# FrancisTheCat/raytracing_c

Measured on AMD Instinct MI355X. Metric: Mray/s, higher is better.
Workload: dtype f32; 1 GPU; helmet.glb 1920x1080, 256 spp, 8 bounces (BASELINE.json configs[2]); partition=single GPU

## Files before the change

include/rt_hip_diag.h:

```cpp
#ifndef RT_HIP_DIAG_H
#define RT_HIP_DIAG_H

#include "rt_hip.h"

#ifdef __cplusplus
extern "C" {
#endif

extern void rt_diag_set_tokens(void *disney_proc, void *debug_proc, void *background_proc);

extern void rt_diag_multi_fault(i32 no_peer, i32 failing_slot);

extern int  rt_set_pipeline(i32 pipeline);
extern i32  rt_get_pipeline(void);
extern void rt_set_wavefront_capacity(i64 records);

extern int rt_get_ledger(u64 *out, i32 n);
extern int rt_get_wave_times(u64 *out, i32 max_waves);
extern i64 rt_diag_device_bytes_live(void);
extern int rt_diag_release_staging(void);


extern int rt_test_math(i32 op, i32 n, f32 const *x, f32 const *y, f32 *out);
extern int rt_test_rcp_sweep(u64 out[6]);
extern int rt_test_srgb_sweep(u64 out[3]);
extern int rt_test_quantize_sweep(u64 out[2]);
extern int rt_test_group_sum(i32 group, i32 n_waves, u64 const *in, u8 const *valid, u64 *out);
extern int rt_test_sky_add_group(void);

extern int rt_test_trace(RT_Device_Scene *dscene, i32 n, f32 const *rays,
                         f32 *out_t, i32 *out_tri, f32 *out_uv);

extern int rt_test_trace_stream(RT_Device_Scene *dscene, i32 n, f32 const *rays, f32 const *pyramid, i32 exit_lanes, i32 mode,
                                f32 *out_t, i32 *out_tri, f32 *out_uv, u64 visits[2]);

extern int rt_test_tile_order(i32 n_tiles, u32 const *cost, u32 *order);

extern int rt_test_texture(RT_Device_Scene *dscene, i32 tex, i32 n, f32 const *uv, f32 *out_rgb);


extern int rt_test_shade(RT_Device_Scene *dscene, i32 mode, i32 n, i32 const *tri, f32 const *in, u32 const *state_in,
                         f32 *out, u32 *state_out, i32 *terminate, i32 *textured);
extern int rt_test_brdf(i32 n, f32 const *params, f32 const *in_dir, u32 const *state_in, f32 *out_dir, f32 *brdf, u32 *state_out);
extern int rt_test_background(RT_Device_Scene *dscene, i32 mode, i32 n, f32 const *dir, f32 *rgb);
extern int rt_test_primary_ray(Camera const *camera, i32 width, i32 height, i32 n, i32 const *xys, f32 *rays);

#ifdef __cplusplus
}
#endif

#endif
```

raytracing_c_amd/csrc/rt_dev.hip.h:

```cpp
#ifndef RT_DEV_HIP_H
#define RT_DEV_HIP_H

#include <hip/hip_runtime.h>
#include <stdint.h>

#include "rt_device.h"
#include "../../include/rt_math.h"

#define RT_BLOCK_WAVES 4
#define RT_BLOCK_THREADS (RT_BLOCK_WAVES * 64)

struct Ray3 {
  rt_v3 o, d;
  float inv_x, inv_y, inv_z;
  bool  fast;
};

__device__ __forceinline__ rt_v3 slab_bias3(const Ray3 &r) {
#ifdef RT_MATH_NO_FMA
  return rt_v3_make(0.0f, 0.0f, 0.0f);
#else
  float px, py, pz;
  asm volatile("v_mul_f32 %0, %1, %2" : "=v"(px) : "v"(r.o.x), "v"(r.inv_x));
  asm volatile("v_mul_f32 %0, %1, %2" : "=v"(py) : "v"(r.o.y), "v"(r.inv_y));
// ... 17 lines not shown
  LG_REGEN_X, LG_REGEN_L, LG_START_X, LG_START_L, LG_PRIM_X, LG_PRIM_L, LG_TILE_X, LG_JOIN_X, LG_FLUSH_X, LG_GRAB_X, LG_ROUND_X, LG_TRAV_CALLS,
  LG_NFULL_X, LG_NFULL_L, LG_NFULL_CAM, LG_NGLOB_X, LG_NGLOB_L, LG_NEXACT_X, LG_NEXACT_L, LG_CULLMASK_X, LG_PYRCHK_X, LG_NODE_WAIT_L,
  LG_NFEW0_X, LG_NFEW1_X, LG_NFEW2_X, LG_NFEW3_X, LG_NFEW4_X, LG_NFEW0_L, LG_NFEW1_L, LG_NFEW2_L, LG_NFEW3_L, LG_NFEW4_L,
  LG_LEAF_X, LG_LEAF_L, LG_LEAF_CAM, LG_POP_X, LG_POP_L, LG_POP_UP_L, LG_POP_RETEST_L, LG_POP_CAM, LG_POP_UP_X, LG_POP_RETEST_X, LG_POP_DONE_L,
  LG_CYC_S, LG_CYC_NODE, LG_CYC_LEAF, LG_CYC_POP, LG_CYC_WAVE, LG_CYC_TILE,
  LG_SKY_X, LG_SKY_L, LG_CYC_SKY,
  LG_CYC_COPY, LG_CYC_JOIN, LG_CYC_DRAIN, LG_DRAIN_X, LG_DRAIN_L, LG_CYC_FLUSH,
  LG_ROOT_FULL_X, LG_ROOT_FULL_L, LG_ROOT_CULL_X, LG_ROOT_CULL_L, LG_ROOT_LEFT_X, LG_ROOT_LEFT_L, LG_ROOTF_X, LG_ROOTF_L,
  LG_N
};
#define RT_LEDGER_ROW 128
#ifdef RT_LEDGER
__device__ __forceinline__ int lane_now();
__device__ __forceinline__ void lg_add(uint32_t *lg, int slot, uint32_t n) {
  if (lg && lane_now() == 0 && n != 0u) __hip_atomic_fetch_add(lg + slot, n, __ATOMIC_RELAXED, __HIP_MEMORY_SCOPE_AGENT);
}
#define LG(slot, n) lg_add(lg, (slot), (uint32_t)(n))
#define LG_ARG , lg
#else
#define LG(slot, n) ((void)0)
#define LG_ARG
#endif
#ifdef RT_LEDGER_MARKS
#define LGM(name) asm volatile("; LEDGER_MARK " name)
#else
#define LGM(name) ((void)0)
#endif
#if defined(RT_LEDGER) && RT_LEDGER >= 2
#define LGT0() const unsigned long long lg_t0 = __builtin_amdgcn_s_memtime()
#define LGT1(slot) LG((slot), (uint32_t)((__builtin_amdgcn_s_memtime() - lg_t0) >> 4))
#define LGD0(n_live) do { if (!lg_drain_t0) { lg_drain_t0 = __builtin_amdgcn_s_memtime(); LG(LG_DRAIN_X, 1); LG(LG_DRAIN_L, (n_live)); } } while (0)
#define LGD1() do { if (lg_drain_t0) { LG(LG_CYC_DRAIN, (uint32_t)((__builtin_amdgcn_s_memtime() - lg_drain_t0) >> 4)); lg_drain_t0 = 0ull; } } while (0)
#else
#define LGT0() ((void)0)
#define LGT1(slot) ((void)0)
#define LGD0(n_live) ((void)0)
#define LGD1() ((void)0)
#endif

__device__ __forceinline__ float4 ld4(const float *base, int idx4) {
  return reinterpret_cast<const float4 *>(base)[idx4];
}

typedef const float __attribute__((address_space(4))) cfloat;
__device__ __forceinline__ cfloat *as_scalar_ptr(const float *p) { return (cfloat *)(unsigned long long)p; }

__device__ __forceinline__ float as_f(int i) { return __int_as_float(i); }
__device__ __forceinline__ int   as_i(float f) { return __float_as_int(f); }


__device__ __forceinline__ float fmin_hw(float a, float b) { return __builtin_fminf(a, b); }
__device__ __forceinline__ float fmax_hw(float a, float b) { return __builtin_fmaxf(a, b); }

template <bool FAST>
__device__ __forceinline__ float slab_entry(const Ray3 &r, const rt_v3 &bs, float mnx, float mny, float mnz,
                                            float mxx, float mxy, float mxz, float t_max) {
  if (FAST) {
    float t0x = rt_slab_t_fast(mnx, r.o.x, r.inv_x, bs.x), t1x = rt_slab_t_fast(mxx, r.o.x, r.inv_x, bs.x);
    float t0y = rt_slab_t_fast(mny, r.o.y, r.inv_y, bs.y), t1y = rt_slab_t_fast(mxy, r.o.y, r.inv_y, bs.y);
    float t0z = rt_slab_t_fast(mnz, r.o.z, r.inv_z, bs.z), t1z = rt_slab_t_fast(mxz, r.o.z, r.inv_z, bs.z);
    float sx = fmin_hw(t0x, t1x), sy = fmin_hw(t0y, t1y), sz = fmin_hw(t0z, t1z);
    float bx = fmax_hw(t0x, t1x), by = fmax_hw(t0y, t1y), bz = fmax_hw(t0z, t1z);
    float t_minv = fmax_hw(RT_EPS, fmax_hw(sx, fmax_hw(sy, sz)));
    float t_maxv = fmin_hw(t_max, fmin_hw(bx, fmin_hw(by, bz)));
    return (t_minv < t_maxv) ? t_minv : RT_INF;
  } else {
    float t0x = rt_slab_t_exact(mnx, r.o.x, r.inv_x), t1x = rt_slab_t_exact(mxx, r.o.x, r.inv_x);
    float t0y = rt_slab_t_exact(mny, r.o.y, r.inv_y), t1y = rt_slab_t_exact(mxy, r.o.y, r.inv_y);
    float t0z = rt_slab_t_exact(mnz, r.o.z, r.inv_z), t1z = rt_slab_t_exact(mxz, r.o.z, r.inv_z);
    float sx = rt_min_ps(t0x, t1x), sy = rt_min_ps(t0y, t1y), sz = rt_min_ps(t0z, t1z);
    float bx = rt_max_ps(t0x, t1x), by = rt_max_ps(t0y, t1y), bz = rt_max_ps(t0z, t1z);
    float t_minv = rt_max_ps(RT_EPS, rt_max_ps(sx, rt_max_ps(sy, sz)));
    float t_maxv = rt_min_ps(t_max, rt_min_ps(bx, rt_min_ps(by, bz)));
    float e = (t_minv >= t_maxv) ? RT_INF : t_minv;
    return (e < t_max) ? e : RT_INF;
  }
}

template <bool FAST>
__device__ __forceinline__ float slab_entry_child(const float *n, const Ray3 &r) {
  float mnx = n[0], mny = n[8], mnz = n[16], mxx = n[24], mxy = n[32], mxz = n[40];
  if (FAST) {
    const rt_v3 bs = slab_bias3(r);
    float t0x = rt_slab_t_fast(mnx, r.o.x, r.inv_x, bs.x), t1x = rt_slab_t_fast(mxx, r.o.x, r.inv_x, bs.x);
    float t0y = rt_slab_t_fast(mny, r.o.y, r.inv_y, bs.y), t1y = rt_slab_t_fast(mxy, r.o.y, r.inv_y, bs.y);
    float t0z = rt_slab_t_fast(mnz, r.o.z, r.inv_z, bs.z), t1z = rt_slab_t_fast(mxz, r.o.z, r.inv_z, bs.z);
    float sx = fmin_hw(t0x, t1x), sy = fmin_hw(t0y, t1y), sz = fmin_hw(t0z, t1z);
    return fmax_hw(RT_EPS, fmax_hw(sx, fmax_hw(sy, sz)));
  }
  float t0x = rt_slab_t_exact(mnx, r.o.x, r.inv_x), t1x = rt_slab_t_exact(mxx, r.o.x, r.inv_x);
  float t0y = rt_slab_t_exact(mny, r.o.y, r.inv_y), t1y = rt_slab_t_exact(mxy, r.o.y, r.inv_y);
  float t0z = rt_slab_t_exact(mnz, r.o.z, r.inv_z), t1z = rt_slab_t_exact(mxz, r.o.z, r.inv_z);
  float sx = rt_min_ps(t0x, t1x), sy = rt_min_ps(t0y, t1y), sz = rt_min_ps(t0z, t1z);
  return rt_max_ps(RT_EPS, rt_max_ps(sx, rt_max_ps(sy, sz)));
}
__device__ __forceinline__ float slab_entry_child_any(const float *n, const Ray3 &r) {
  if (r.fast) return slab_entry_child<true>(n, r);
  return slab_entry_child<false>(n, r);
}

#define NODE_GLOBAL 0
#define NODE_SCALAR 1
#define NODE_LDS_ORDERED 3
#define RT_LDS_NODE_F4 13

static_assert(RT_LDS_NODE_F4 * 16 == RT_LDS_NODE_BYTES, "the host splits the LDS by the kernels' node stride (rt_device.h, lds_split)");

__device__ __forceinline__ int lds_node_f4(int node) { return (int)__umul24((unsigned)node, (unsigned)RT_LDS_NODE_F4); }

static inline int raise_lds_limit(const void *kernel, uint32_t *devices, int smem_bytes, int limit) {
  int dev = 0;
  (void)hipGetDevice(&dev);
  if (smem_bytes > 48 * 1024 && (dev >= 32 || !(__atomic_load_n(devices, __ATOMIC_RELAXED) & (1u << dev)))) {
    hipError_t e = hipFuncSetAttribute(kernel, hipFuncAttributeMaxDynamicSharedMemorySize, limit);
    if (e != hipSuccess) return (int)e;
    if (dev < 32) __atomic_fetch_or(devices, 1u << dev, __ATOMIC_RELAXED);
  }
  return 0;
}

template <bool FAST, int MODE>
__device__ __forceinline__ uint32_t node_enter(const RT_KParams &P, const Ray3 &r, int node, float hit_t,
                                               const float4 *lds_nodes) {
  int d[8];
  const rt_v3 bs = FAST ? slab_bias3(r) : rt_v3_make(0.0f, 0.0f, 0.0f);
  if (MODE == NODE_SCALAR) {
    cfloat *nb = as_scalar_ptr(P.nodes) + (size_t)node * 48;
#pragma unroll
    for (int k = 0; k < 8; k++) {
      d[k] = as_i(slab_entry<FAST>(r, bs, nb[k], nb[8 + k], nb[16 + k], nb[24 + k], nb[32 + k], nb[40 + k], hit_t));
    }
  } else if (MODE == NODE_LDS_ORDERED) {
    static_assert(FAST || MODE != NODE_LDS_ORDERED, "the ordered LDS form is for FAST rays only");
    const char *nbase = reinterpret_cast<const char *>(lds_nodes + lds_node_f4(node));
    const int nx = (as_i(r.inv_x) >> 31) & 96, ny = (as_i(r.inv_y) >> 31) & 96, nz = (as_i(r.inv_z) >> 31) & 96;
#pragma unroll
    for (int h = 0; h < 2; h++) {
      const float4 ax = *reinterpret_cast<const float4 *>(nbase + nx + h * 16), bx = *reinterpret_cast<const float4 *>(nbase + (96 - nx) + h * 16);
      const float4 ay = *reinterpret_cast<const float4 *>(nbase + 32 + ny + h * 16), by = *reinterpret_cast<const float4 *>(nbase + 32 + (96 - ny) + h * 16);
      const float4 az = *reinterpret_cast<const float4 *>(nbase + 64 + nz + h * 16), bz = *reinterpret_cast<const float4 *>(nbase + 64 + (96 - nz) + h * 16);
      const float nxs[4] = {ax.x, ax.y, ax.z, ax.w}, fxs[4] = {bx.x, bx.y, bx.z, bx.w};
      const float nys[4] = {ay.x, ay.y, ay.z, ay.w}, fys[4] = {by.x, by.y, by.z, by.w};
      const float nzs[4] = {az.x, az.y, az.z, az.w}, fzs[4] = {bz.x, bz.y, bz.z, bz.w};
#pragma unroll
      for (int k = 0; k < 4; k++) {
        const float sx = rt_slab_t_fast(nxs[k], r.o.x, r.inv_x, bs.x), bxx = rt_slab_t_fast(fxs[k], r.o.x, r.inv_x, bs.x);
        const float sy = rt_slab_t_fast(nys[k], r.o.y, r.inv_y, bs.y), byy = rt_slab_t_fast(fys[k], r.o.y, r.inv_y, bs.y);
        const float sz = rt_slab_t_fast(nzs[k], r.o.z, r.inv_z, bs.z), bzz = rt_slab_t_fast(fzs[k], r.o.z, r.inv_z, bs.z);
        const float t_minv = fmax_hw(RT_EPS, fmax_hw(sx, fmax_hw(sy, sz)));
        const float t_maxv = fmin_hw(hit_t, fmin_hw(bxx, fmin_hw(byy, bzz)));
        d[h * 4 + k] = as_i((t_minv < t_maxv) ? t_minv : RT_INF);
      }
    }
  } else {
    const float4 *nb = reinterpret_cast<const float4 *>(P.nodes) + (size_t)node * 12;
#pragma unroll
    for (int h = 0; h < 2; h++) {
      float4 mnx = nb[0 + h], mny = nb[2 + h], mnz = nb[4 + h];
      float4 mxx = nb[6 + h], mxy = nb[8 + h], mxz = nb[10 + h];
      d[h * 4 + 0] = as_i(slab_entry<FAST>(r, bs, mnx.x, mny.x, mnz.x, mxx.x, mxy.x, mxz.x, hit_t));
      d[h * 4 + 1] = as_i(slab_entry<FAST>(r, bs, mnx.y, mny.y, mnz.y, mxx.y, mxy.y, mxz.y, hit_t));
      d[h * 4 + 2] = as_i(slab_entry<FAST>(r, bs, mnx.z, mny.z, mnz.z, mxx.z, mxy.z, mxz.z, hit_t));
      d[h * 4 + 3] = as_i(slab_entry<FAST>(r, bs, mnx.w, mny.w, mnz.w, mxx.w, mxy.w, mxz.w, hit_t));
    }
  }

  int rank[8];
#pragma unroll
  for (int k = 0; k < 8; k++) rank[k] = k;
#pragma unroll
  for (int j = 0; j < 8; j++) {
#pragma unroll
    for (int k = j + 1; k < 8; k++) {
      int kb = (int)((uint32_t)(d[k] - d[j]) >> 31);
      rank[j] += kb;
      rank[k] -= kb;
    }
  }
  uint32_t w = 0, n_inf = 0;
#pragma unroll
  for (int j = 0; j < 8; j++) {
    int sh;
    asm("v_lshl_add_u32 %0, %1, 1, %1" : "=v"(sh) : "v"(rank[j]));
    w |= (uint32_t)j << sh;
    n_inf += ((uint32_t)d[j] + 0x00800000u) >> 31;
  }
  return w | ((8u - n_inf) << 24);
}

#define RT_SHORT_DIV_MAX_X 0x1p102f
__device__ __forceinline__ float rcp_exact(float x) {
  float xs = x * 0x1p24f;
  float y = __builtin_amdgcn_rcpf(xs);
  float e = __builtin_fmaf(-xs, y, 1.0f);
  float z = __builtin_fmaf(e, y, y);
  return __builtin_amdgcn_div_fixupf(z, xs, 1.0f) * 0x1p24f;
}
__device__ __forceinline__ float rcp_leaf(float x) {
  float xs = x * 0x1p24f;
  float y = __builtin_amdgcn_rcpf(xs);
  float e = __builtin_fmaf(-xs, y, 1.0f);
  float z = __builtin_fmaf(e, y, y);
  return z * 0x1p24f;
}
__device__ __forceinline__ bool rcp_exact_outside(float x) {
  return __builtin_fabsf(x) >= RT_SHORT_DIV_MAX_X && __builtin_fabsf(x) < RT_INF;
}

__device__ __forceinline__ rt_v3 normalize_dev(rt_v3 v) { return rt_v3_scale(v, rcp_exact(rt_sqrtf(rt_v3_dot(v, v)))); }

__device__ __forceinline__ unsigned long long accum_quantize_dev(float c) {
  float v = (c > 0.0f) ? c : 0.0f;
  v = (v > RT_ACCUM_MAX) ? RT_ACCUM_MAX : v;
  const uint32_t b = __float_as_uint(v);
  const uint32_t e = b >> 23;
  const unsigned long long m = (unsigned long long)((b & 0x007FFFFFu) | 0x00800000u) << 29;
  const uint32_t k = 147u - e;
  return m >> (k < 63u ? k : 63u);
}

__device__ __forceinline__ float tri_test(const Ray3 &r, float ax, float ay, float az, float e1x, float e1y, float e1z,
                                          float e2x, float e2y, float e2z, float &u_out, float &v_out) {
  rt_v3 a = rt_v3_make(ax, ay, az);
  rt_v3 edge1 = rt_v3_make(e1x, e1y, e1z);
  rt_v3 edge2 = rt_v3_make(e2x, e2y, e2z);
  rt_v3 rxe2 = rt_v3_cross(r.d, edge2);
  float det = rt_v3_dot(edge1, rxe2);
  float inv_det = 1.0f / det;
  rt_v3 s = rt_v3_sub(r.o, a);
  rt_v3 sxe1 = rt_v3_cross(s, edge1);
  float u = inv_det * rt_v3_dot(s, rxe2);
  float v = inv_det * rt_v3_dot(r.d, sxe1);
  float t = inv_det * rt_v3_dot(edge2, sxe1);
  bool miss = (u < -RT_EPS) || (u > 1.0f + RT_EPS) || (v < -RT_EPS) || (u + v > 1.0f + RT_EPS) || (t < RT_EPS);
  float dist = miss ? RT_INF : t;
  u_out = u;
  v_out = v;
  return (dist > 0.0f) ? dist : RT_INF;
}

// ... 1179 lines not shown
```

raytracing_c_amd/csrc/rt_diag.cpp:

```cpp

#include "rt_host.h"

#include <cmath>

#ifndef RT_DIAG_VARIANTS
#error rt_diag.cpp belongs to the diagnostic library only (-DRT_DIAG_VARIANTS)
#endif

extern "C" {
int rt_launch_test_math(int op, int n, const float *x, const float *y, float *out, hipStream_t stream);
int rt_launch_test_rcp_sweep(unsigned long long *counts, hipStream_t stream);
int rt_launch_test_srgb_sweep(unsigned long long *counts, hipStream_t stream);
int rt_launch_test_quantize_sweep(unsigned long long *counts, hipStream_t stream);
int rt_launch_test_sky_add_group(void);
int rt_launch_test_group_sum(int group, int n_waves, const unsigned long long *in, const unsigned char *valid, unsigned long long *out,
                              hipStream_t stream);
int rt_launch_test_trace(const RT_KParams *P, int n, const float *rays, float *out_t, int *out_tri, float *out_uv,
                         hipStream_t stream);
int rt_launch_test_trace_stream(const RT_KParams *P, int n, const float *rays, const float *pyr, int exit_lanes, int n_blocks,
                                int smem_bytes, float *out_t, int *out_tri, float *out_uv, unsigned long long *visits,
                                hipStream_t stream);
int rt_launch_test_texture(const RT_KParams *P, int tex, int n, const float *uv, float *out, hipStream_t stream);
int rt_launch_test_shade(const RT_KParams *P, int lds, int n, const int *tri, const float *in, const uint32_t *state_in, float *out,
                         uint32_t *state_out, int *terminate, int *textured, hipStream_t stream);
int rt_launch_test_brdf(int n, const float *params, const float *in_dir, const uint32_t *state_in, float *out_dir, float *brdf,
                        uint32_t *state_out, hipStream_t stream);
int rt_launch_test_background(const RT_KParams *P, int lds, int n, const float *dir, float *rgb, hipStream_t stream);
int rt_launch_test_primary_ray(const RT_KParams *P, int n, const int *xys, float *rays, hipStream_t stream);
int rt_wf_launch_camera(const RT_KParams *P, int n_blocks, int geometry, int smem_bytes, hipStream_t stream);
int rt_wf_launch_trace(const RT_KParams *P, int n_blocks, int geometry, int smem_bytes, hipStream_t stream);
int rt_wf_launch_shade(const RT_KParams *P, int n_blocks, int first, hipStream_t stream);
}

std::atomic<int>            g_pipeline{0};
static std::atomic<int64_t> g_wf_cap_records{(int64_t)96 << 20};

extern "C" int rt_set_pipeline(i32 pipeline) {
  if (pipeline != 0 && pipeline != 1) return rt_fail("rt_set_pipeline: %d is not 0 (tile stream) or 1 (wavefront)", pipeline);
  g_pipeline.store(pipeline);
  return 0;
}
extern "C" i32 rt_get_pipeline(void) { return g_pipeline.load(); }
extern "C" void rt_set_wavefront_capacity(i64 records) {
  if (records >= 1024) g_wf_cap_records.store(records);
}

extern "C" void rt_diag_set_tokens(void *disney, void *debug, void *background) {
  if (disney) g_tok_disney = (Shader_Proc)disney;
  if (debug) g_tok_debug = (Shader_Proc)debug;
  if (background) g_tok_background = (Background_Proc)background;
}

static int wavefront_ensure_queues(RT_Device_Scene *d, int64_t paths, int cam_waves, int max_waves) {
  const int64_t cap = g_wf_cap_records.load();
  const int64_t want = paths < cap ? paths : cap;
  const int64_t fill = WF_CHUNK - 63;
  const int64_t soft = (want + fill - 1) / fill + cam_waves + 1;
  if (d->wf_ctl && d->wf_soft0 >= soft && d->wf_waves >= max_waves) return 0;
  d->wf_hit0.reset(); d->wf_hit.reset(); d->wf_ray[0].reset(); d->wf_ray[1].reset(); d->wf_cnt.reset(); d->wf_ctl.reset();
  d->wf_soft0 = 0;
  const int64_t hard = soft + 2 * (int64_t)cam_waves + 8;
  const int64_t ray_chunks = (hard * WF_CHUNK + fill - 1) / fill + max_waves + 8;
  const int64_t hit_chunks = (ray_chunks * WF_CHUNK + fill - 1) / fill + max_waves + 8;
  HIP_TRY(d->wf_hit0.grow((size_t)hard * WF_HIT0_FIELDS * WF_CHUNK));
  HIP_TRY(d->wf_hit.grow((size_t)hit_chunks * WF_HIT_FIELDS * WF_CHUNK));
  HIP_TRY(d->wf_ray[0].grow((size_t)ray_chunks * WF_RAY_FIELDS * WF_CHUNK));
  HIP_TRY(d->wf_ray[1].grow((size_t)ray_chunks * WF_RAY_FIELDS * WF_CHUNK));
  HIP_TRY(d->wf_cnt.grow((size_t)(hard + hit_chunks + 2 * ray_chunks)));
  HIP_TRY(d->wf_ctl.grow((size_t)WF_N_CTL * WF_CTL_STRIDE));
// ... 116 lines not shown
  HIP_TRY(dout.grow((size_t)n));
  HIP_TRY(hipMemcpy(dx, x, bytes, hipMemcpyHostToDevice));
  if (y) {
    HIP_TRY(dy.grow((size_t)n));
    HIP_TRY(hipMemcpy(dy, y, bytes, hipMemcpyHostToDevice));
  }
  int rc = rt_launch_test_math(op, n, dx, dy, dout, nullptr);
  if (rc == 0) rc = (int)hipMemcpy(out, dout, bytes, hipMemcpyDeviceToHost);
  if (rc != 0) return rt_fail("rt_test_math failed: %s", hipGetErrorString((hipError_t)rc));
  return 0;
}

static int run_sweep(int (*launch)(unsigned long long *, hipStream_t), const char *name, u64 *out, int n_out) {
  Device &D = dev0();
  std::lock_guard<std::mutex> lock(D.mutex);
  if (ensure_device(D) != 0) return -1;
  if (!out) return rt_fail("%s: NULL", name);
  DevMem<unsigned long long> b;
  HIP_TRY(b.grow((size_t)n_out));
  HIP_TRY(hipMemset(b, 0, (size_t)n_out * sizeof(unsigned long long)));
  int rc = launch(b, nullptr);
  if (rc == 0) rc = (int)hipMemcpy(out, b, (size_t)n_out * sizeof(unsigned long long), hipMemcpyDeviceToHost);
  if (rc != 0) return rt_fail("%s failed: %s", name, hipGetErrorString((hipError_t)rc));
  return 0;
}

extern "C" int rt_test_rcp_sweep(u64 out[6]) { return run_sweep(rt_launch_test_rcp_sweep, "rt_test_rcp_sweep", out, 6); }

extern "C" int rt_test_srgb_sweep(u64 out[3]) { return run_sweep(rt_launch_test_srgb_sweep, "rt_test_srgb_sweep", out, 3); }

extern "C" int rt_test_quantize_sweep(u64 out[2]) { return run_sweep(rt_launch_test_quantize_sweep, "rt_test_quantize_sweep", out, 2); }

extern "C" int rt_test_group_sum(i32 group, i32 n_waves, u64 const *in, u8 const *valid, u64 *out) {
  Device &D = dev0();
  std::lock_guard<std::mutex> lock(D.mutex);
  if (ensure_device(D) != 0) return -1;
  if ((group != 4 && group != 16 && group != 64) || n_waves <= 0 || n_waves > 65535 || !in || !valid || !out)
    return rt_fail("rt_test_group_sum: bad arguments");
  const size_t n = (size_t)n_waves * 64;
  DevMem<unsigned long long> din, dout;
  DevMem<unsigned char> dvalid;
  HIP_TRY(din.grow(3 * n));
  HIP_TRY(dout.grow(3 * n));
  HIP_TRY(dvalid.grow(n));
  HIP_TRY(hipMemcpy(din, in, 3 * n * sizeof(u64), hipMemcpyHostToDevice));
  HIP_TRY(hipMemcpy(dvalid, valid, n, hipMemcpyHostToDevice));
  int rc = rt_launch_test_group_sum(group, n_waves, din, dvalid, dout, nullptr);
  if (rc == 0) rc = (int)hipMemcpy(out, dout, 3 * n * sizeof(u64), hipMemcpyDeviceToHost);
  if (rc != 0) return rt_fail("rt_test_group_sum failed: %s", hipGetErrorString((hipError_t)rc));
  return 0;
}

extern "C" int rt_test_sky_add_group(void) { return rt_launch_test_sky_add_group(); }

extern "C" int rt_test_tile_order(i32 n_tiles, u32 const *cost, u32 *order) {
  Device &D = dev0();
  std::lock_guard<std::mutex> lock(D.mutex);
  if (ensure_device(D) != 0) return -1;
  if (n_tiles <= 0 || !cost || !order) return rt_fail("rt_test_tile_order: bad arguments");
  DevMem<uint32_t> bc, bo, bn, bw, bz;
  DevMem<unsigned long long> bk;
  HIP_TRY(bc.grow((size_t)n_tiles));
  HIP_TRY(bo.grow((size_t)n_tiles));
  HIP_TRY(bn.grow((size_t)n_tiles + (size_t)(n_tiles + 63) / 64));
  HIP_TRY(bk.grow(RT_N_COUNTERS));
  HIP_TRY(bw.grow(16));
  HIP_TRY(bz.grow((size_t)n_tiles));
  HIP_TRY(hipMemcpy(bc, cost, (size_t)n_tiles * 4, hipMemcpyHostToDevice));
  HIP_TRY(hipMemset(bo, 0xFF, (size_t)n_tiles * 4));
  int rc = rt_launch_prepare(n_tiles, bn, bn + n_tiles, bk, bw, bz, bc, bo, nullptr);
  if (rc == 0) rc = (int)hipMemcpy(order, bo, (size_t)n_tiles * 4, hipMemcpyDeviceToHost);
  if (rc != 0) return rt_fail("rt_test_tile_order failed: %s", hipGetErrorString((hipError_t)rc));
  return 0;
}

extern "C" int rt_test_trace(RT_Device_Scene *d, i32 n, f32 const *rays, f32 *out_t, i32 *out_tri, f32 *out_uv) {
  if (!d || n <= 0 || !rays || !out_t || !out_tri || !out_uv) return rt_fail("rt_test_trace: bad arguments");
  Device &D = *d->dev;
  std::lock_guard<std::mutex> lock(D.mutex);
  DeviceGuard guard(D);
  if (ensure_device(D) != 0) return -1;
  RT_KParams K;
  scene_only_kparams(&K, d);
  DevMem<float> dr, dt, duv;
  DevMem<int>   dtri;
  HIP_TRY(dr.grow((size_t)n * 6));
  HIP_TRY(dt.grow((size_t)n));
  HIP_TRY(dtri.grow((size_t)n));
  HIP_TRY(duv.grow((size_t)n * 2));
  HIP_TRY(hipMemcpy(dr, rays, (size_t)n * 24, hipMemcpyHostToDevice));
  int rc = rt_launch_test_trace(&K, n, dr, dt, dtri, duv, nullptr);
  if (rc == 0) rc = (int)hipMemcpy(out_t, dt, (size_t)n * 4, hipMemcpyDeviceToHost);
  if (rc == 0) rc = (int)hipMemcpy(out_tri, dtri, (size_t)n * 4, hipMemcpyDeviceToHost);
  if (rc == 0) rc = (int)hipMemcpy(out_uv, duv, (size_t)n * 8, hipMemcpyDeviceToHost);
  if (rc != 0) return rt_fail("rt_test_trace failed: %s", hipGetErrorString((hipError_t)rc));
  return 0;
}

extern "C" int rt_test_trace_stream(RT_Device_Scene *d, i32 n, f32 const *rays, f32 const *pyramid, i32 exit_lanes, i32 mode,
                                    f32 *out_t, i32 *out_tri, f32 *out_uv, u64 visits[2]) {
  if (!d || n <= 0 || !rays || !out_t || !out_tri || !out_uv || !visits) return rt_fail("rt_test_trace_stream: bad arguments");
  if (exit_lanes < 1 || exit_lanes > 64) return rt_fail("rt_test_trace_stream: exit_lanes %d outside [1, 64]", exit_lanes);
  Device &D = *d->dev;
  std::lock_guard<std::mutex> lock(D.mutex);
  DeviceGuard guard(D);
  if (ensure_device(D) != 0) return -1;
// ... 166 lines not shown
```

raytracing_c_amd/ctypes_abi.py:

```python
import ctypes as C

import numpy as np

isize = C.c_ssize_t
f32 = C.c_float


class Vec2(C.Structure):
    _fields_ = [("x", f32), ("y", f32)]


class Vec3(C.Structure):
    _fields_ = [("x", f32), ("y", f32), ("z", f32)]


class Matrix_4x4(C.Structure):
    _fields_ = [("rows", (f32 * 4) * 4)]


class Byte_Slice(C.Structure):
    _fields_ = [("data", C.c_void_p), ("len", isize)]


class Image(C.Structure):
# ... 151 lines not shown
    _fields_ = [("sigma_normal", f32), ("sigma_position", f32)]


assert C.sizeof(RT_Variance_Params) == 8
RT_TEMPORAL_MOMENTS_PER_PIXEL = 16


RAY_HIT_DTYPE = np.dtype([("t", "<f4"), ("triangle", "<i4"), ("u", "<f4"), ("v", "<f4")])
_HIT_HEAD = [("distance", "<f4"), ("normal", "<f4", (3,)), ("normal_geo", "<f4", (3,)), ("point", "<f4", (3,)),
             ("tangent", "<f4", (3,)), ("bitangent", "<f4", (3,)), ("tex_coords", "<f4", (2,))]
DEVICE_HIT_DTYPE = np.dtype(_HIT_HEAD + [("triangle", "<i4"), ("material", "<i4"), ("pad", "<i4", (2,))])
HIT_DTYPE = np.dtype(_HIT_HEAD + [("shader_data", "<u8"), ("shader_proc", "<u8")])
assert RAY_HIT_DTYPE.itemsize == C.sizeof(RT_Ray_Hit) == 16
assert DEVICE_HIT_DTYPE.itemsize == C.sizeof(RT_Device_Hit) == 88
assert HIT_DTYPE.itemsize == C.sizeof(Hit) == 88
RT_QUERY_MAX_RAYS = 1 << 30
RT_QUERY_SLICE = 1 << 20

assert C.sizeof(BVH_Node) == 192
assert C.sizeof(Triangle) == 112
assert C.sizeof(Triangle_AOS) == 112
assert C.sizeof(Hit) == 88
assert C.sizeof(PBR_Shader_Data) == 80

TRIANGLE_DTYPE = np.dtype([("positions", "<f4", (3, 3)), ("normals", "<f4", (3, 3)), ("tex_coords", "<f4", (3, 2)),
                           ("shader_data", "<u8"), ("shader_proc", "<u8")])
assert TRIANGLE_DTYPE.itemsize == 112

EXPORTED_SYMBOLS = [
    "render_thread_proc", "rendering_context_is_finished", "rendering_context_finish", "lightmap_bake", "render",
    "denoise_image",
    "scene_init", "scene_init_sah", "scene_init_gpu", "rt_scene_alloc", "rt_scene_free", "scene_load_bytes", "scene_save_bytes", "scene_file_size",
    "rt_scene_slot_map", "scene_refit", "scene_refit_gpu",
    "disney_shader_proc", "debug_shader_proc", "sample_background",
    "rt_last_error", "rt_clear_error", "rt_init", "rt_set_seed", "rt_get_seed",
    "rt_set_devices", "rt_device_count", "rt_math_contract",
    "rt_scene_verify", "rt_scene_touch", "rt_scene_set_static", "rt_get_frame_timing",
    "rt_scene_upload", "rt_scene_release", "rt_scene_invalidate", "rt_scene_device_bytes", "rt_set_camera",
    "rt_chunk_count", "rt_chunk_owner", "rt_local_chunk_count", "rt_max_local_chunk_count", "rt_local_chunk_list", "rt_render_accumulate", "rt_resolve", "rt_untile",
    "rt_denoise", "rt_render_frame", "rt_frame_begin", "rt_frame_end", "rt_render_views", "rt_render_accumulate_views",
    "rt_query_closest", "rt_query_occluded", "rt_scene_hits", "rt_scene_closest", "rt_scene_occluded", "rt_get_query_counters",
    "rt_render_accumulate_features", "rt_resolve_features", "rt_render_features",
    "rt_guided_work_bytes", "rt_guided_denoise", "rt_guided_denoise_host", "rt_render_denoised",
    "rt_temporal_history_bytes", "rt_temporal_accumulate", "rt_temporal_accumulate_host", "rt_history_create", "rt_history_reset",
    "rt_history_destroy", "rt_render_temporal",
    "rt_temporal_moments_bytes", "rt_temporal_accumulate_moments", "rt_temporal_accumulate_moments_host",
    "rt_guided_variance_work_bytes", "rt_guided_denoise_variance", "rt_guided_denoise_variance_host", "rt_render_svgf",
    "rt_get_counters", "rt_get_skipped_root_visits", "rt_get_leafless_paths", "rt_get_fused_root_visits", "rt_last_kernel_ms", "rt_kernel_timing_reset", "rt_kernel_timing_mean_ms",
]

DIAG_ONLY_SYMBOLS = [
    "rt_diag_set_tokens", "rt_diag_multi_fault", "rt_set_pipeline", "rt_get_pipeline", "rt_set_wavefront_capacity", "rt_get_wave_times", "rt_get_ledger",
    "rt_diag_device_bytes_live", "rt_diag_release_staging",
    "rt_test_math", "rt_test_rcp_sweep", "rt_test_srgb_sweep", "rt_test_quantize_sweep", "rt_test_group_sum", "rt_test_sky_add_group", "rt_test_trace", "rt_test_trace_stream",
    "rt_test_tile_order", "rt_test_texture", "rt_test_shade", "rt_test_brdf", "rt_test_background", "rt_test_primary_ray",
]
```

raytracing_c_amd/native.py:

```python
import ctypes as C
import os

from . import ctypes_abi as abi

_HERE = os.path.dirname(os.path.abspath(__file__))
LIB_PATH = os.environ.get("RT_LIB_PATH") or os.path.join(_HERE, "librt_hip.so")
DIAG_PATH = os.path.join(_HERE, "librt_hip_diag.so")


class NativeLibraryMissing(RuntimeError):
    pass


def _preload_hip_runtime():
    import importlib.util
    import sys
    if os.environ.get("RT_HIP_RUNTIME", "torch") != "torch":
        return
    if "torch" in sys.modules:
        return
    try:
        spec = importlib.util.find_spec("torch")
    except (ImportError, ValueError):
        spec = None
# ... 124 lines not shown
        d.rt_temporal_moments_bytes.restype = C.c_int64
        d.rt_temporal_accumulate_moments.argtypes = ([C.c_int32, C.c_int32, P(abi.RT_Temporal_Params), P(abi.Camera), P(abi.Camera)]
                                                     + [vp] * 10 + [P(abi.RT_Variance_Params)] + [vp] * 4)
        d.rt_temporal_accumulate_moments_host.argtypes = [C.c_int32, C.c_int32, P(abi.RT_Temporal_Params), P(abi.Camera), P(abi.Camera),
                                                          vp, P(abi.RT_Features), P(abi.RT_History_Planes), P(abi.RT_History_Planes),
                                                          vp, vp, vp, P(abi.RT_Variance_Params), vp, vp, vp]
        d.rt_guided_variance_work_bytes.argtypes = [C.c_int32, C.c_int32]
        d.rt_guided_variance_work_bytes.restype = C.c_int64
        d.rt_guided_denoise_variance.argtypes = [C.c_int32, C.c_int32, P(abi.RT_Guided_Params)] + [vp] * 11
        d.rt_guided_denoise_variance_host.argtypes = [C.c_int32, C.c_int32, P(abi.RT_Guided_Params), vp, P(abi.RT_Features), vp, vp, vp,
                                                      vp]
        d.rt_render_svgf.argtypes = [P(abi.Scene), P(abi.Image), abi.isize, abi.isize, vp, P(abi.RT_Temporal_Params),
                                     P(abi.RT_Variance_Params), P(abi.RT_Guided_Params), vp, vp, vp, vp]
    d.rt_get_counters.argtypes = [P(abi.RT_Counters)]
    if hasattr(d, "rt_get_skipped_root_visits"):
        d.rt_get_skipped_root_visits.argtypes = [P(C.c_uint64)]
    if hasattr(d, "rt_get_leafless_paths"):
        d.rt_get_leafless_paths.argtypes = [P(C.c_uint64)]
    if hasattr(d, "rt_get_fused_root_visits"):
        d.rt_get_fused_root_visits.argtypes = [P(C.c_uint64)]
    d.rt_math_contract.restype = C.c_int
    d.rt_last_kernel_ms.restype = C.c_float
    d.rt_kernel_timing_reset.restype = None
    d.rt_kernel_timing_mean_ms.argtypes = [P(C.c_int32)]
    d.rt_kernel_timing_mean_ms.restype = C.c_float
    d.rt_set_devices.argtypes = [C.c_int32, C.c_int32]
    d.rt_device_count.restype = C.c_int32
    d.rt_scene_verify.argtypes = [P(abi.Scene)]
    d.rt_scene_touch.argtypes = [P(abi.Scene), vp, C.c_size_t]
    d.rt_scene_set_static.argtypes = [P(abi.Scene), C.c_int32]
    d.rt_scene_set_static.restype = None
    d.rt_get_frame_timing.argtypes = [P(abi.RT_Frame_Timing)]
    d.render_thread_proc.argtypes = [P(abi.Rendering_Context)]
    d.render_thread_proc.restype = None
    d.rendering_context_is_finished.argtypes = [P(abi.Rendering_Context)]
    d.rendering_context_is_finished.restype = C.c_bool
    d.rendering_context_finish.argtypes = [P(abi.Rendering_Context)]
    d.rendering_context_finish.restype = None
    d.render.argtypes = [P(abi.Scene), P(abi.Image), abi.isize, abi.isize]
    d.lightmap_bake.argtypes = [P(abi.Image), P(abi.Scene), abi.isize]
    d.lightmap_bake.restype = None
    d.denoise_image.argtypes = [P(abi.Image), P(abi.Image), abi.isize]
    d.denoise_image.restype = None
    d.rt_denoise.argtypes = [C.c_int32, C.c_int32, vp, vp, vp]


def _declare_diag(d):
    vp = C.c_void_p
    d.rt_test_math.argtypes = [C.c_int32, C.c_int32, vp, vp, vp]
    d.rt_test_rcp_sweep.argtypes = [vp]
    d.rt_test_srgb_sweep.argtypes = [vp]
    d.rt_test_quantize_sweep.argtypes = [vp]
    d.rt_test_group_sum.argtypes = [C.c_int32, C.c_int32, vp, vp, vp]
    d.rt_test_trace.argtypes = [vp, C.c_int32, vp, vp, vp, vp]
    d.rt_test_texture.argtypes = [vp, C.c_int32, C.c_int32, vp, vp]
    d.rt_test_shade.argtypes = [vp, C.c_int32, C.c_int32] + [vp] * 7
    d.rt_test_brdf.argtypes = [C.c_int32] + [vp] * 6
    d.rt_test_background.argtypes = [vp, C.c_int32, C.c_int32, vp, vp]
    d.rt_test_primary_ray.argtypes = [C.POINTER(abi.Camera), C.c_int32, C.c_int32, C.c_int32, vp, vp]
    d.rt_test_trace_stream.argtypes = [vp, C.c_int32, vp, vp, C.c_int32, C.c_int32, vp, vp, vp, vp]
    d.rt_test_tile_order.argtypes = [C.c_int32, vp, vp]
    d.rt_set_pipeline.argtypes = [C.c_int32]
    d.rt_get_pipeline.restype = C.c_int32
    d.rt_set_wavefront_capacity.argtypes = [C.c_int64]
    d.rt_set_wavefront_capacity.restype = None
    d.rt_get_wave_times.argtypes = [vp, C.c_int32]
    d.rt_get_ledger.argtypes = [vp, C.c_int32]
    d.rt_diag_device_bytes_live.argtypes = []
    d.rt_diag_device_bytes_live.restype = C.c_int64
    d.rt_diag_release_staging.argtypes = []
    d.rt_diag_multi_fault.argtypes = [C.c_int32, C.c_int32]
    d.rt_diag_multi_fault.restype = None
    d.rt_diag_set_tokens.argtypes = [vp, vp, vp]
    d.rt_diag_set_tokens.restype = None


lib = _Lazy(LIB_PATH)
diag = _Lazy(DIAG_PATH, diag=True)


def symbol_address(name):
    return C.cast(getattr(lib, name), C.c_void_p).value


def last_error(which=None):
    return ((which or lib).rt_last_error() or b"").decode("utf-8", "replace")
```

Before: 22820 Mray/s.

## Order BVH children with a packed-key sorting network instead of pairwise rank counting

For fast rays, each child's entry distance is packed into a 32-bit key: the float bits offset from RT_EPS, shifted left by three, with the child index in the low bits. The eight keys are then ordered with a 19-comparator sorting network, and the child order is extracted with alignbit, replacing the 28 pairwise compares and rank accumulation. If any lane's distances overflow the key range, the wave falls back to the original rank-based ordering. This is meant to cut VALU work per node visit, at the cost of more live registers and a rarely taken fallback path. A diagnostic test entry point for the new ordering is also added.

```diff
diff --git a/include/rt_hip_diag.h b/include/rt_hip_diag.h
--- a/include/rt_hip_diag.h
+++ b/include/rt_hip_diag.h
@@ -27,6 +27,7 @@
 extern int rt_test_quantize_sweep(u64 out[2]);
 extern int rt_test_group_sum(i32 group, i32 n_waves, u64 const *in, u8 const *valid, u64 *out);
 extern int rt_test_sky_add_group(void);
+extern int rt_test_node_order(i32 n, u32 const *t_min, u8 const *cand, u32 *out);
 
 extern int rt_test_trace(RT_Device_Scene *dscene, i32 n, f32 const *rays,
                          f32 *out_t, i32 *out_tri, f32 *out_uv);
diff --git a/raytracing_c_amd/csrc/rt_dev.hip.h b/raytracing_c_amd/csrc/rt_dev.hip.h
--- a/raytracing_c_amd/csrc/rt_dev.hip.h
+++ b/raytracing_c_amd/csrc/rt_dev.hip.h
@@ -93,18 +93,26 @@
 __device__ __forceinline__ float fmin_hw(float a, float b) { return __builtin_fminf(a, b); }
 __device__ __forceinline__ float fmax_hw(float a, float b) { return __builtin_fmaxf(a, b); }
 
+__device__ __forceinline__ float slab_entry_fast(const Ray3 &r, const rt_v3 &bs, float mnx, float mny, float mnz,
+                                                 float mxx, float mxy, float mxz, float t_max, bool &cand) {
+  float t0x = rt_slab_t_fast(mnx, r.o.x, r.inv_x, bs.x), t1x = rt_slab_t_fast(mxx, r.o.x, r.inv_x, bs.x);
+  float t0y = rt_slab_t_fast(mny, r.o.y, r.inv_y, bs.y), t1y = rt_slab_t_fast(mxy, r.o.y, r.inv_y, bs.y);
+  float t0z = rt_slab_t_fast(mnz, r.o.z, r.inv_z, bs.z), t1z = rt_slab_t_fast(mxz, r.o.z, r.inv_z, bs.z);
+  float sx = fmin_hw(t0x, t1x), sy = fmin_hw(t0y, t1y), sz = fmin_hw(t0z, t1z);
+  float bx = fmax_hw(t0x, t1x), by = fmax_hw(t0y, t1y), bz = fmax_hw(t0z, t1z);
+  float t_minv = fmax_hw(RT_EPS, fmax_hw(sx, fmax_hw(sy, sz)));
+  float t_maxv = fmin_hw(t_max, fmin_hw(bx, fmin_hw(by, bz)));
+  cand = t_minv < t_maxv;
+  return t_minv;
+}
+
 template <bool FAST>
 __device__ __forceinline__ float slab_entry(const Ray3 &r, const rt_v3 &bs, float mnx, float mny, float mnz,
                                             float mxx, float mxy, float mxz, float t_max) {
   if (FAST) {
-    float t0x = rt_slab_t_fast(mnx, r.o.x, r.inv_x, bs.x), t1x = rt_slab_t_fast(mxx, r.o.x, r.inv_x, bs.x);
-    float t0y = rt_slab_t_fast(mny, r.o.y, r.inv_y, bs.y), t1y = rt_slab_t_fast(mxy, r.o.y, r.inv_y, bs.y);
-    float t0z = rt_slab_t_fast(mnz, r.o.z, r.inv_z, bs.z), t1z = rt_slab_t_fast(mxz, r.o.z, r.inv_z, bs.z);
-    float sx = fmin_hw(t0x, t1x), sy = fmin_hw(t0y, t1y), sz = fmin_hw(t0z, t1z);
-    float bx = fmax_hw(t0x, t1x), by = fmax_hw(t0y, t1y), bz = fmax_hw(t0z, t1z);
-    float t_minv = fmax_hw(RT_EPS, fmax_hw(sx, fmax_hw(sy, sz)));
-    float t_maxv = fmin_hw(t_max, fmin_hw(bx, fmin_hw(by, bz)));
-    return (t_minv < t_maxv) ? t_minv : RT_INF;
+    bool cand;
+    const float t_minv = slab_entry_fast(r, bs, mnx, mny, mnz, mxx, mxy, mxz, t_max, cand);
+    return cand ? t_minv : RT_INF;
   } else {
     float t0x = rt_slab_t_exact(mnx, r.o.x, r.inv_x), t1x = rt_slab_t_exact(mxx, r.o.x, r.inv_x);
     float t0y = rt_slab_t_exact(mny, r.o.y, r.inv_y), t1y = rt_slab_t_exact(mxy, r.o.y, r.inv_y);
@@ -160,16 +168,91 @@
   return 0;
 }
 
-template <bool FAST, int MODE>
-__device__ __forceinline__ uint32_t node_enter(const RT_KParams &P, const Ray3 &r, int node, float hit_t,
-                                               const float4 *lds_nodes) {
+#define RT_KEY_BASE    0x38D1B717u
+#define RT_KEY_MISS    0xFFFFFFF8u
+#define RT_KEY_RAW_END 0x1FFFFFFFu
+static_assert(__builtin_bit_cast(uint32_t, RT_EPS) == RT_KEY_BASE, "the keys count from the bit pattern of RT_EPS");
+static_assert(((RT_KEY_RAW_END - 1u) << 3 | 7u) < RT_KEY_MISS && (RT_KEY_RAW_END << 3) == RT_KEY_MISS, "the largest exact key is below the miss keys");
+
+struct NodeKeys {
+  uint32_t key[8];
+  uint32_t max_raw;
+  uint32_t n_cand;
+};
+__device__ __forceinline__ void node_key_put(NodeKeys &K, int k, float t_minv, bool cand) {
+  const uint32_t raw = __float_as_uint(t_minv) - RT_KEY_BASE;
+  K.max_raw = raw > K.max_raw ? raw : K.max_raw;
+  K.key[k] = cand ? ((raw << 3) | (uint32_t)k) : (RT_KEY_MISS | (uint32_t)k);
+  K.n_cand += cand ? 1u : 0u;
+}
+__device__ __forceinline__ bool node_keys_exact(const NodeKeys &K) { return K.max_raw < RT_KEY_RAW_END; }
+
+#define RT_KEY_CMPX(a, b) do { const uint32_t lo_ = K.key[a] < K.key[b] ? K.key[a] : K.key[b], hi_ = K.key[a] < K.key[b] ? K.key[b] : K.key[a]; \
+                               K.key[a] = lo_; K.key[b] = hi_; } while (0)
+__device__ __forceinline__ uint32_t node_order_keys(NodeKeys &K) {
+  RT_KEY_CMPX(0, 2); RT_KEY_CMPX(1, 3); RT_KEY_CMPX(4, 6); RT_KEY_CMPX(5, 7);
+  RT_KEY_CMPX(0, 4); RT_KEY_CMPX(1, 5); RT_KEY_CMPX(2, 6); RT_KEY_CMPX(3, 7);
+  RT_KEY_CMPX(0, 1); RT_KEY_CMPX(2, 3); RT_KEY_CMPX(4, 5); RT_KEY_CMPX(6, 7);
+  RT_KEY_CMPX(2, 4); RT_KEY_CMPX(3, 5);
+  RT_KEY_CMPX(1, 4); RT_KEY_CMPX(3, 6);
+  RT_KEY_CMPX(1, 2); RT_KEY_CMPX(3, 4); RT_KEY_CMPX(5, 6);
+  uint32_t w = 0;
+#pragma unroll
+  for (int m = 0; m < 8; m++) w = __builtin_amdgcn_alignbit(K.key[m], w, 3);
+  return (w >> 8) | (K.n_cand << 24);
+}
+#undef RT_KEY_CMPX
+
+__device__ __forceinline__ uint32_t node_order_rank(const int (&d)[8]) {
+  int rank[8];
+#pragma unroll
+  for (int k = 0; k < 8; k++) rank[k] = k;
+#pragma unroll
+  for (int j = 0; j < 8; j++) {
+#pragma unroll
+    for (int k = j + 1; k < 8; k++) {
+      int kb = (int)((uint32_t)(d[k] - d[j]) >> 31);
+      rank[j] += kb;
+      rank[k] -= kb;
+    }
+  }
+  uint32_t w = 0, n_inf = 0;
+#pragma unroll
+  for (int j = 0; j < 8; j++) {
+    int sh;
+    asm("v_lshl_add_u32 %0, %1, 1, %1" : "=v"(sh) : "v"(rank[j]));
+    w |= (uint32_t)j << sh;
+    n_inf += ((uint32_t)d[j] + 0x00800000u) >> 31;
+  }
+  return w | ((8u - n_inf) << 24);
+}
+
+template <bool KEYED>
+__device__ __forceinline__ void node_child_put(NodeKeys &K, int (&d)[8], int k, float t_minv, bool cand) {
+  if (KEYED) node_key_put(K, k, t_minv, cand);
+  else d[k] = as_i(cand ? t_minv : RT_INF);
+}
+
+template <bool FAST, int MODE, bool KEYED>
+__device__ __forceinline__ uint32_t node_enter_form(const RT_KParams &P, const Ray3 &r, int node, float hit_t,
+                                                    const float4 *lds_nodes, bool &exact) {
+  static_assert(FAST || !KEYED, "keys are for the FAST slab forms only");
   int d[8];
+  NodeKeys K;
+  K.max_raw = 0u;
+  K.n_cand = 0u;
   const rt_v3 bs = FAST ? slab_bias3(r) : rt_v3_make(0.0f, 0.0f, 0.0f);
   if (MODE == NODE_SCALAR) {
     cfloat *nb = as_scalar_ptr(P.nodes) + (size_t)node * 48;
 #pragma unroll
     for (int k = 0; k < 8; k++) {
-      d[k] = as_i(slab_entry<FAST>(r, bs, nb[k], nb[8 + k], nb[16 + k], nb[24 + k], nb[32 + k], nb[40 + k], hit_t));
+      if (FAST) {
+        bool cand;
+        const float t_minv = slab_entry_fast(r, bs, nb[k], nb[8 + k], nb[16 + k], nb[24 + k], nb[32 + k], nb[40 + k], hit_t, cand);
+        node_child_put<KEYED>(K, d, k, t_minv, cand);
+      } else {
+        d[k] = as_i(slab_entry<false>(r, bs, nb[k], nb[8 + k], nb[16 + k], nb[24 + k], nb[32 + k], nb[40 + k], hit_t));
+      }
     }
   } else if (MODE == NODE_LDS_ORDERED) {
     static_assert(FAST || MODE != NODE_LDS_ORDERED, "the ordered LDS form is for FAST rays only");
@@ -190,7 +273,7 @@
         const float sz = rt_slab_t_fast(nzs[k], r.o.z, r.inv_z, bs.z), bzz = rt_slab_t_fast(fzs[k], r.o.z, r.inv_z, bs.z);
         const float t_minv = fmax_hw(RT_EPS, fmax_hw(sx, fmax_hw(sy, sz)));
         const float t_maxv = fmin_hw(hit_t, fmin_hw(bxx, fmin_hw(byy, bzz)));
-        d[h * 4 + k] = as_i((t_minv < t_maxv) ? t_minv : RT_INF);
+        node_child_put<KEYED>(K, d, h * 4 + k, t_minv, t_minv < t_maxv);
       }
     }
   } else {
@@ -199,34 +282,37 @@
     for (int h = 0; h < 2; h++) {
       float4 mnx = nb[0 + h], mny = nb[2 + h], mnz = nb[4 + h];
       float4 mxx = nb[6 + h], mxy = nb[8 + h], mxz = nb[10 + h];
-      d[h * 4 + 0] = as_i(slab_entry<FAST>(r, bs, mnx.x, mny.x, mnz.x, mxx.x, mxy.x, mxz.x, hit_t));
-      d[h * 4 + 1] = as_i(slab_entry<FAST>(r, bs, mnx.y, mny.y, mnz.y, mxx.y, mxy.y, mxz.y, hit_t));
-      d[h * 4 + 2] = as_i(slab_entry<FAST>(r, bs, mnx.z, mny.z, mnz.z, mxx.z, mxy.z, mxz.z, hit_t));
-      d[h * 4 + 3] = as_i(slab_entry<FAST>(r, bs, mnx.w, mny.w, mnz.w, mxx.w, mxy.w, mxz.w, hit_t));
-    }
-  }
-
-  int rank[8];
-#pragma unroll
-  for (int k = 0; k < 8; k++) rank[k] = k;
-#pragma unroll
-  for (int j = 0; j < 8; j++) {
-#pragma unroll
-    for (int k = j + 1; k < 8; k++) {
-      int kb = (int)((uint32_t)(d[k] - d[j]) >> 31);
-      rank[j] += kb;
-      rank[k] -= kb;
-    }
-  }
-  uint32_t w = 0, n_inf = 0;
-#pragma unroll
-  for (int j = 0; j < 8; j++) {
-    int sh;
-    asm("v_lshl_add_u32 %0, %1, 1, %1" : "=v"(sh) : "v"(rank[j]));
-    w |= (uint32_t)j << sh;
-    n_inf += ((uint32_t)d[j] + 0x00800000u) >> 31;
-  }
-  return w | ((8u - n_inf) << 24);
+      const float c_mnx[4] = {mnx.x, mnx.y, mnx.z, mnx.w}, c_mny[4] = {mny.x, mny.y, mny.z, mny.w}, c_mnz[4] = {mnz.x, mnz.y, mnz.z, mnz.w};
+      const float c_mxx[4] = {mxx.x, mxx.y, mxx.z, mxx.w}, c_mxy[4] = {mxy.x, mxy.y, mxy.z, mxy.w}, c_mxz[4] = {mxz.x, mxz.y, mxz.z, mxz.w};
+#pragma unroll
+      for (int k = 0; k < 4; k++) {
+        if (FAST) {
+          bool cand;
+          const float t_minv = slab_entry_fast(r, bs, c_mnx[k], c_mny[k], c_mnz[k], c_mxx[k], c_mxy[k], c_mxz[k], hit_t, cand);
+          node_child_put<KEYED>(K, d, h * 4 + k, t_minv, cand);
+        } else {
+          d[h * 4 + k] = as_i(slab_entry<false>(r, bs, c_mnx[k], c_mny[k], c_mnz[k], c_mxx[k], c_mxy[k], c_mxz[k], hit_t));
+        }
+      }
+    }
+  }
+  if (KEYED) {
+    exact = node_keys_exact(K);
+    return node_order_keys(K);
+  }
+  exact = true;
+  return node_order_rank(d);
+}
+
+template <bool FAST, int MODE>
+__device__ __forceinline__ uint32_t node_enter(const RT_KParams &P, const Ray3 &r, int node, float hit_t,
+                                               const float4 *lds_nodes) {
+  bool exact;
+  const uint32_t w = node_enter_form<FAST, MODE, FAST>(P, r, node, hit_t, lds_nodes, exact);
+  if (!FAST || __builtin_expect(__ballot(!exact) == 0ull, 1)) return w;
+  if (MODE == NODE_SCALAR) asm volatile("" : "+s"(node));
+  else asm volatile("" : "+v"(node));
+  return node_enter_form<FAST, MODE, false>(P, r, node, hit_t, lds_nodes, exact);
 }
 
 #define RT_SHORT_DIV_MAX_X 0x1p102f
diff --git a/raytracing_c_amd/csrc/rt_diag.cpp b/raytracing_c_amd/csrc/rt_diag.cpp
--- a/raytracing_c_amd/csrc/rt_diag.cpp
+++ b/raytracing_c_amd/csrc/rt_diag.cpp
@@ -15,6 +15,7 @@
 int rt_launch_test_sky_add_group(void);
 int rt_launch_test_group_sum(int group, int n_waves, const unsigned long long *in, const unsigned char *valid, unsigned long long *out,
                               hipStream_t stream);
+int rt_launch_test_node_order(int n, const uint32_t *t_min, const unsigned char *cand, uint32_t *out, hipStream_t stream);
 int rt_launch_test_trace(const RT_KParams *P, int n, const float *rays, float *out_t, int *out_tri, float *out_uv,
                          hipStream_t stream);
 int rt_launch_test_trace_stream(const RT_KParams *P, int n, const float *rays, const float *pyr, int exit_lanes, int n_blocks,
@@ -237,6 +238,24 @@
 }
 
 extern "C" int rt_test_sky_add_group(void) { return rt_launch_test_sky_add_group(); }
+
+extern "C" int rt_test_node_order(i32 n, u32 const *t_min, u8 const *cand, u32 *out) {
+  Device &D = dev0();
+  std::lock_guard<std::mutex> lock(D.mutex);
+  if (ensure_device(D) != 0) return -1;
+  if (n <= 0 || n > (1 << 24) || !t_min || !cand || !out) return rt_fail("rt_test_node_order: bad arguments");
+  DevMem<uint32_t> dt, dout;
+  DevMem<unsigned char> dcand;
+  HIP_TRY(dt.grow((size_t)n * 8));
+  HIP_TRY(dcand.grow((size_t)n * 8));
+  HIP_TRY(dout.grow((size_t)n * 3));
+  HIP_TRY(hipMemcpy(dt, t_min, (size_t)n * 8 * sizeof(u32), hipMemcpyHostToDevice));
+  HIP_TRY(hipMemcpy(dcand, cand, (size_t)n * 8, hipMemcpyHostToDevice));
+  int rc = rt_launch_test_node_order(n, dt, dcand, dout, nullptr);
+  if (rc == 0) rc = (int)hipMemcpy(out, dout, (size_t)n * 3 * sizeof(u32), hipMemcpyDeviceToHost);
+  if (rc != 0) return rt_fail("rt_test_node_order failed: %s", hipGetErrorString((hipError_t)rc));
+  return 0;
+}
 
 extern "C" int rt_test_tile_order(i32 n_tiles, u32 const *cost, u32 *order) {
   Device &D = dev0();
diff --git a/raytracing_c_amd/ctypes_abi.py b/raytracing_c_amd/ctypes_abi.py
--- a/raytracing_c_amd/ctypes_abi.py
+++ b/raytracing_c_amd/ctypes_abi.py
@@ -227,6 +227,6 @@
 DIAG_ONLY_SYMBOLS = [
     "rt_diag_set_tokens", "rt_diag_multi_fault", "rt_set_pipeline", "rt_get_pipeline", "rt_set_wavefront_capacity", "rt_get_wave_times", "rt_get_ledger",
     "rt_diag_device_bytes_live", "rt_diag_release_staging",
-    "rt_test_math", "rt_test_rcp_sweep", "rt_test_srgb_sweep", "rt_test_quantize_sweep", "rt_test_group_sum", "rt_test_sky_add_group", "rt_test_trace", "rt_test_trace_stream",
+    "rt_test_math", "rt_test_rcp_sweep", "rt_test_srgb_sweep", "rt_test_quantize_sweep", "rt_test_group_sum", "rt_test_sky_add_group", "rt_test_node_order", "rt_test_trace", "rt_test_trace_stream",
     "rt_test_tile_order", "rt_test_texture", "rt_test_shade", "rt_test_brdf", "rt_test_background", "rt_test_primary_ray",
 ]
diff --git a/raytracing_c_amd/native.py b/raytracing_c_amd/native.py
--- a/raytracing_c_amd/native.py
+++ b/raytracing_c_amd/native.py
@@ -200,6 +200,7 @@
     d.rt_test_srgb_sweep.argtypes = [vp]
     d.rt_test_quantize_sweep.argtypes = [vp]
     d.rt_test_group_sum.argtypes = [C.c_int32, C.c_int32, vp, vp, vp]
+    d.rt_test_node_order.argtypes = [C.c_int32, vp, vp, vp]
     d.rt_test_trace.argtypes = [vp, C.c_int32, vp, vp, vp, vp]
     d.rt_test_texture.argtypes = [vp, C.c_int32, C.c_int32, vp, vp]
     d.rt_test_shade.argtypes = [vp, C.c_int32, C.c_int32] + [vp] * 7
```

After: 23360 Mray/s (median of 6 runs). 1.02x the previous value.
